# tbuckworth/train-procgen-pytorch

Hardware: AMD Instinct MI355X
Metric: env steps/sec (whole node), coinrun hard-500 IMPALA-CNN PPO (higher is better)
Workload: dtype bf16

## Files before the change

### scratch/kbench_cb.hip

```cpp
#include "conv_bf16.hip"
#include <cstdio>
#include <vector>
int main(int argc, char** argv) {
    const int n = argc > 1 ? atoi(argv[1]) : 8192, reps = 10;
    const size_t P = (size_t)n * 16 * 16 * 32, X = (size_t)n * 32 * 32 * 16;
    unsigned short *dp, *xi, *out, *bank; uint8_t* arg; float* slabs;
    hipMalloc(&dp, P * 2 + 4096); hipMalloc(&arg, P + 4096); hipMalloc(&xi, X * 2 + 4096); hipMalloc(&out, X * 2 + 4096);
    hipMalloc(&bank, 16 * 304 * 2 + 4096); hipMalloc(&slabs, (size_t)1024 * (4608 + 32) * 4);
    std::vector<unsigned short> h(X);
    for (size_t k = 0; k < X; ++k) h[k] = (unsigned short)((k * 2654435761u >> 16) & 0xBFFF);
    hipMemcpy(dp, h.data(), P * 2, hipMemcpyHostToDevice); hipMemcpy(xi, h.data(), X * 2, hipMemcpyHostToDevice);
    std::vector<uint8_t> ha(P);
    for (size_t k = 0; k < P; ++k) ha[k] = (uint8_t)((k * 40503u >> 7) % 9);
    hipMemcpy(arg, ha.data(), P, hipMemcpyHostToDevice);
    std::vector<unsigned short> hb(16 * 304, 0x3c00); hipMemcpy(bank, hb.data(), hb.size() * 2, hipMemcpyHostToDevice);
    hipStream_t st; hipStreamCreate(&st);
    hipEvent_t e0, e1; hipEventCreate(&e0); hipEventCreate(&e1);
    ConvArgs a{};
    a.in = dp; a.pool_arg = arg; a.out = out; a.n = n; a.bf16 = 1; a.wbank = bank; a.wg_in = xi; a.wg_partial = slabs;
    auto run = [&]() { launch_conv_dgrad_bf16(CS_16_32_32, a, st); };
    run(); hipStreamSynchronize(st);
#ifdef BF_TIMING
    unsigned long long zero[16] = {0}; hipMemcpyToSymbol(HIP_SYMBOL(g_bf_timing), zero, sizeof zero);
#endif
    hipEventRecord(e0, st);
    for (int r = 0; r < reps; ++r) run();
    hipEventRecord(e1, st); hipStreamSynchronize(st);
    float ms; hipEventElapsedTime(&ms, e0, e1);
    const int grid = conv_bwd_fused_grid(CS_16_32_32, n);
    printf("fused block2.conv backward n=%d grid=%d: %.1f us/launch  (%s)\n", n, grid, ms * 1000 / reps, hipGetErrorString(hipGetLastError()));
#ifdef BF_TIMING
    unsigned long long t[16]; hipMemcpyFromSymbol(t, HIP_SYMBOL(g_bf_timing), sizeof t);
    const char* nm[8] = {"top barrier (+ wait for loads)", "staging stores + barrier", "gather (+ next loads)", "barrier after gather", "wgrad MFMAs", "dgrad MFMAs", "tail: reduction + slab", "prologue"};
    for (int role = 0; role < 2; ++role)
        for (int k = 0; k < 8; ++k) printf("  wave %d %-32s %9.0f cycles/WG/launch (%.0f per item)\n", role * 4, nm[k], (double)t[role * 8 + k] / grid / reps, (double)t[role * 8 + k] / grid / reps / ((double)n * 4 / grid));
#endif
    return 0;
}
```

### train-procgen-pytorch_amd/csrc/conv_bf16.hip

```cpp
#include "common.h"
#include "device_util.h"
#include <mutex>
#include <type_traits>

static int c1_grid(int n);


template <int CH, int HO, int NPR>
struct PoolStage {
    static constexpr int NW = NPR * HO * (CH / 8), K = (NW + 255) / 256;
    static constexpr int PD_ELEMS = NPR * HO * CH;
    static constexpr size_t BYTES = (size_t)PD_ELEMS * 3;
    uint4 rd[K]; uint2 ra[K];
    __device__ __forceinline__ void load(const unsigned short* g_dp, const uint8_t* g_arg, long long img, int oyb) {
#pragma unroll
        for (int k = 0; k < K; ++k) {
            const int e = threadIdx.x + k * 256;
            rd[k] = (uint4){0u, 0u, 0u, 0u}; ra[k] = (uint2){0xffffffffu, 0xffffffffu};
            if (e < NW) {
                const int c8 = e % (CH / 8), ox = (e / (CH / 8)) % HO, oy = oyb + e / ((CH / 8) * HO);
                if (oy >= 0 && oy < HO) {
                    const long long o = ((img * HO + oy) * HO + ox) * CH + c8 * 8;
                    rd[k] = *(const uint4*)(g_dp + o); ra[k] = *(const uint2*)(g_arg + o);
                }
            }
        }
    }
    __device__ __forceinline__ void store(unsigned short* s_pd) const {
        uint8_t* s_pa = (uint8_t*)(s_pd + PD_ELEMS);
#pragma unroll
        for (int k = 0; k < K; ++k) {
            const int e = threadIdx.x + k * 256;
            if (e < NW) { *(uint4*)(s_pd + e * 8) = rd[k]; *(uint2*)(s_pa + e * 8) = ra[k]; }
        }
    }
    static __device__ __forceinline__ void gather(const unsigned short* s_pd, int a0, int y_lo, int y_hi, unsigned short* s_dst, int y_base,
                                                  int dst_pw, int xoff, int S) {
        for (int task = threadIdx.x; task < NTASK; task += 256) gather_task(s_pd, task, a0, y_lo, y_hi, s_dst, y_base, dst_pw, xoff, S);
    }
    static constexpr int NTASK = (NPR - 1) * HO * (CH / 4);
    static __device__ __forceinline__ void gather_task(const unsigned short* s_pd, int task, int a0, int y_lo, int y_hi, unsigned short* s_dst,
                                                       int y_base, int dst_pw, int xoff, int S) {
        const uint8_t* s_pa = (const uint8_t*)(s_pd + PD_ELEMS);
        constexpr int Q = CH / 4;
        {
            const int cq = task % Q, bx = (task / Q) % HO, bl = task / (Q * HO);
            float sm[4][4];
#pragma unroll
            for (int q = 0; q < 4; ++q)
#pragma unroll
                for (int c = 0; c < 4; ++c) sm[q][c] = 0.f;
#pragma unroll
            for (int wy = 0; wy < 2; ++wy)
#pragma unroll
                for (int wx = 0; wx < 2; ++wx) {
                    const int ox = bx + wx;
                    const int o = ((bl + wy) * HO + (ox < HO ? ox : HO - 1)) * CH + cq * 4;
                    const uint2 d = *(const uint2*)(s_pd + o);
                    unsigned ag = *(const unsigned*)(s_pa + o);
                    if (ox >= HO) ag = 0xffffffffu;
                    const float v[4] = {__uint_as_float(d.x << 16), __uint_as_float(d.x & 0xffff0000u), __uint_as_float(d.y << 16), __uint_as_float(d.y & 0xffff0000u)};
#pragma unroll
                    for (int dy = 0; dy < 2; ++dy)
#pragma unroll
                        for (int dx = 0; dx < 2; ++dx) {
                            const int ky = dy + 1 - 2 * wy, kx = dx + 1 - 2 * wx;
                            if (ky < 0 || kx < 0) continue;
                            const unsigned pos = (unsigned)(ky * 3 + kx);
#pragma unroll
                            for (int c = 0; c < 4; ++c)
                                sm[dy * 2 + dx][c] += (((ag >> (8 * c)) & 0xffu) == pos) ? v[c] : 0.f;
                        }
                }
#pragma unroll
            for (int dy = 0; dy < 2; ++dy) {
                const int y = 2 * (a0 + bl) + dy;
                if (y < y_lo || y >= y_hi) continue;
#pragma unroll
                for (int dx = 0; dx < 2; ++dx) {
                    const float* q = sm[dy * 2 + dx];
                    *(uint2*)(s_dst + ((y - y_base) * dst_pw + 2 * bx + dx + xoff) * S + cq * 4) =
                        (uint2){mi_pk_bf16(q[0], q[1]), mi_pk_bf16(q[2], q[3])};
                }
            }
        }
    }
    static constexpr int NTASK2 = (NPR - 1) * HO * (CH / 2);
    static __device__ __forceinline__ void gather_task2(const unsigned short* s_pd, int task, int a0, int y_lo, int y_hi, unsigned short* s_dst,
                                                        int y_base, int dst_pw, int xoff, int S) {
        const uint8_t* s_pa = (const uint8_t*)(s_pd + PD_ELEMS);
        constexpr int Q = CH / 2;
        const int cq = task % Q, bx = (task / Q) % HO, bl = task / (Q * HO);
        float sm[4][2];
#pragma unroll
        for (int q = 0; q < 4; ++q) { sm[q][0] = 0.f; sm[q][1] = 0.f; }
#pragma unroll
        for (int wy = 0; wy < 2; ++wy)
#pragma unroll
            for (int wx = 0; wx < 2; ++wx) {
                const int ox = bx + wx;
                const int o = ((bl + wy) * HO + (ox < HO ? ox : HO - 1)) * CH + cq * 2;
                const unsigned d = *(const unsigned*)(s_pd + o);
                unsigned ag = *(const unsigned short*)(s_pa + o);
                if (ox >= HO) ag = 0xffffu;
                const float v[2] = {__uint_as_float(d << 16), __uint_as_float(d & 0xffff0000u)};
#pragma unroll
                for (int dy = 0; dy < 2; ++dy)
#pragma unroll
                    for (int dx = 0; dx < 2; ++dx) {
                        const int ky = dy + 1 - 2 * wy, kx = dx + 1 - 2 * wx;
                        if (ky < 0 || kx < 0) continue;
                        const unsigned pos = (unsigned)(ky * 3 + kx);
#pragma unroll
                        for (int c = 0; c < 2; ++c)
                            sm[dy * 2 + dx][c] += (((ag >> (8 * c)) & 0xffu) == pos) ? v[c] : 0.f;
                    }
            }
#pragma unroll
        for (int dy = 0; dy < 2; ++dy) {
            const int y = 2 * (a0 + bl) + dy;
            if (y < y_lo || y >= y_hi) continue;
#pragma unroll
            for (int dx = 0; dx < 2; ++dx)
                *(unsigned*)(s_dst + ((y - y_base) * dst_pw + 2 * bx + dx + xoff) * S + cq * 2) = mi_pk_bf16(sm[dy * 2 + dx][0], sm[dy * 2 + dx][1]);
        }
    }
};

template <int CIN_, int COUT_, int HW_, int TH_, int TW_, int NIMG_, bool TRANSW_>
struct BfCfg {
    static constexpr int CIN = CIN_, COUT = COUT_, HW = HW_, TH = TH_, TW = TW_, NIMG = NIMG_;
    static constexpr bool TRANSW = TRANSW_;
    static constexpr int S = (CIN == 16) ? 16 : 48;
    static constexpr int PH = TH + 2, PW = TW + 2;
    static constexpr int NPIX = NIMG * PH * PW;
    static constexpr int IN_ELEMS = ((NPIX * S + 7) / 8) * 8;
    static constexpr int NK = (CIN == 32) ? 9 : 5;
    static constexpr int WS = NK * 32 + 16;
    static constexpr int W_ELEMS = COUT * WS;
    static constexpr int NMT = NIMG * TH * TW / 16, MT = NMT / 4, NB = COUT / 16;
    static constexpr int TPI_X = HW / TW, TPI = (HW / TH) * (HW / TW);
    static constexpr int C8 = CIN / 8;
    static constexpr int NLD = (NPIX * C8 + 255) / 256;
    static constexpr size_t LDS_BYTES = (size_t)(IN_ELEMS + W_ELEMS) * 2;
    static constexpr int WPE = 1;
    static_assert(NMT % 4 == 0, "M tiles must split over 4 waves");
};

template <class C>
__device__ __forceinline__ void bf_coords(int work, int& img0, int& ty0, int& tx0) {
    if (C::NIMG > 1) { img0 = work * C::NIMG; ty0 = 0; tx0 = 0; }
    else { img0 = work / C::TPI; const int t = work % C::TPI; ty0 = (t / C::TPI_X) * C::TH; tx0 = (t % C::TPI_X) * C::TW; }
}

template <class C>
__device__ __forceinline__ void bf_tile_load(uint4 (&r)[C::NLD], const unsigned short* in, int n_img, int img0, int ty0, int tx0) {
#pragma unroll
    for (int k = 0; k < C::NLD; ++k) {
        const int e = threadIdx.x + k * 256;
        uint4 v = {0u, 0u, 0u, 0u};
        if (e < C::NPIX * C::C8) {
            const int pix = e / C::C8, c8 = e % C::C8;
            const int img = pix / (C::PH * C::PW), q = pix % (C::PH * C::PW);
            const int gy = ty0 + q / C::PW - 1, gx = tx0 + q % C::PW - 1, n = img0 + img;
            if (n < n_img && gy >= 0 && gy < C::HW && gx >= 0 && gx < C::HW)
                v = *(const uint4*)(in + (((long long)n * C::HW + gy) * C::HW + gx) * C::CIN + c8 * 8);
        }
        r[k] = v;
    }
}
__device__ __forceinline__ unsigned relu_bf16x2(unsigned w) {
    const unsigned neg = (w >> 15) & 0x00010001u;
    return w & ~(neg * 0xFFFFu);
}
template <class C>
__device__ __forceinline__ void bf_tile_store(const uint4 (&r)[C::NLD], unsigned short* s_in, int relu_in) {
#pragma unroll
    for (int k = 0; k < C::NLD; ++k) {
        const int e = threadIdx.x + k * 256;
        if (e < C::NPIX * C::C8) {
            uint4 v = r[k];
            if (relu_in) { v.x = relu_bf16x2(v.x); v.y = relu_bf16x2(v.y); v.z = relu_bf16x2(v.z); v.w = relu_bf16x2(v.w); }
            *(uint4*)(s_in + (e / C::C8) * C::S + (e % C::C8) * 8) = v;
        }
    }
}

template <class C, bool POOLIN = false>
__global__ __launch_bounds__(256, C::WPE) void conv3x3_bf16_kernel(ConvArgs a) {
    extern __shared__ __attribute__((aligned(16))) unsigned short smem_h[];
    unsigned short* s_in = smem_h;
    unsigned short* s_w = smem_h + C::IN_ELEMS;
    using PS = PoolStage<C::CIN, C::HW / 2, C::TH / 2 + 3>;
    unsigned short* s_pd = s_w + C::W_ELEMS;
    static_assert(!POOLIN || (C::NIMG == 1 && C::TW == C::HW && C::TH % 2 == 0), "pooled input: full-width row tiles of one image");
    const int tid = threadIdx.x, lane = tid & 63, wave = tid >> 6;
    const int i = lane & 15, kq = lane >> 4;
    const unsigned short* g_in = (const unsigned short*)a.in;
    const unsigned short* g_mask = (const unsigned short*)a.mask;
    const unsigned short* g_res = (const unsigned short*)a.res;
    unsigned short* g_out = (unsigned short*)a.out;

    if (a.wbank) {
        for (int e = tid; e < C::COUT * C::WS / 8; e += 256) ((uint4*)s_w)[e] = ((const uint4*)a.wbank)[e];
    } else
    for (int e = tid; e < C::COUT * C::WS; e += 256) {
        const int j = e / C::WS, k = e % C::WS;
        float v = 0.f;
        const int tap = k / C::CIN, ci = k % C::CIN;
        if (k < C::NK * 32 && tap < 9) v = C::TRANSW ? a.w[(ci * 9 + (8 - tap)) * C::COUT + j] : a.w[(j * 9 + tap) * C::CIN + ci];
        s_w[e] = f2bf(v);
    }

    float bias_r[C::NB][4];
#pragma unroll
    for (int nb = 0; nb < C::NB; ++nb)
#pragma unroll
        for (int r = 0; r < 4; ++r) bias_r[nb][r] = a.bias ? a.bias[nb * 16 + kq * 4 + r] : 0.f;
    int koff[C::NK];
#pragma unroll
    for (int m = 0; m < C::NK; ++m) {
        int tap, chunk;
        if (C::CIN == 32) { tap = m; chunk = kq; } else { tap = 2 * m + (kq >> 1); chunk = kq & 1; if (tap > 8) tap = 8; }
        koff[m] = ((tap / 3) * C::PW + (tap % 3)) * C::S + chunk * 8;
    }

    const int nwork = (C::NIMG > 1) ? (a.n + C::NIMG - 1) / C::NIMG : a.n * C::TPI;
    uint4 regs[POOLIN ? 1 : C::NLD];
    PS ps;
    int img0, ty0, tx0;
    if (POOLIN) for (int e = tid; e < C::IN_ELEMS / 8; e += 256) ((uint4*)s_in)[e] = (uint4){0u, 0u, 0u, 0u};
    if ((int)blockIdx.x < nwork) {
        bf_coords<C>(blockIdx.x, img0, ty0, tx0);
        if constexpr (POOLIN) ps.load(g_in, a.pool_arg, img0, ty0 / 2 - 1); else bf_tile_load<C>(regs, g_in, a.n, img0, ty0, tx0);
    }
    for (int work = blockIdx.x; work < nwork; work += gridDim.x) {
        bf_coords<C>(work, img0, ty0, tx0);
        __syncthreads();
        if constexpr (POOLIN) {
            ps.store(s_pd);
            __syncthreads();
            PS::gather(s_pd, ty0 / 2 - 1, ty0 - 1, ty0 + C::TH + 1, s_in, ty0 - 1, C::PW, 1, C::S);
        } else bf_tile_store<C>(regs, s_in, a.relu_in);
        __syncthreads();
        if (work + (int)gridDim.x < nwork) {
            int i2, y2, x2;
            bf_coords<C>(work + gridDim.x, i2, y2, x2);
            if constexpr (POOLIN) ps.load(g_in, a.pool_arg, i2, y2 / 2 - 1); else bf_tile_load<C>(regs, g_in, a.n, i2, y2, x2);
        }
        uint2 e_mask[C::MT][C::NB], e_res[C::MT][C::NB];
        long long e_off[C::MT];
        bool e_on[C::MT];
#pragma unroll
        for (int mt = 0; mt < C::MT; ++mt) {
            const int pl = (wave * C::MT + mt) * 16 + i, y = pl / C::TW, x = pl % C::TW;
            int n = img0 + y / C::TH;
            e_on[mt] = n < a.n;
            n = n < a.n ? n : a.n - 1;
            e_off[mt] = (((long long)n * C::HW + ty0 + (y % C::TH)) * C::HW + tx0 + x) * C::COUT + kq * 4;
        }
        if (g_mask) {
#pragma unroll
            for (int mt = 0; mt < C::MT; ++mt)
#pragma unroll
                for (int nb = 0; nb < C::NB; ++nb) e_mask[mt][nb] = *(const uint2*)(g_mask + e_off[mt] + nb * 16);
        } else {
#pragma unroll
            for (int mt = 0; mt < C::MT; ++mt)
#pragma unroll
                for (int nb = 0; nb < C::NB; ++nb) e_mask[mt][nb] = (uint2){0x3f803f80u, 0x3f803f80u};
// ... 88 lines not shown
    const int i = lane & 15, kq = lane >> 4;
    const int pair = wave & 3, role = wave >> 2;
#ifdef BF_TIMING
    long long tacc_[8] = {0, 0, 0, 0, 0, 0, 0, 0}, tlast_ = clock64();
#endif
    const unsigned short* g_dp = (const unsigned short*)a.in;
    const unsigned short* g_xi = (const unsigned short*)a.wg_in;
    unsigned short* g_out = (unsigned short*)a.out;

    for (int e = tid; e < C::COUT * C::WS / 8; e += K::NT) ((uint4*)s_w)[e] = ((const uint4*)a.wbank)[e];
    for (int e = tid; e < K::IN_ELEMS / 8; e += K::NT) ((uint4*)s_in)[e] = (uint4){0u, 0u, 0u, 0u};
    for (int e = tid; e < K::XI_ELEMS / 8; e += K::NT) ((uint4*)s_xi)[e] = (uint4){0u, 0u, 0u, 0u};
    for (int e = tid; e < K::ONES_ELEMS / 2; e += K::NT) ((unsigned*)s_ones)[e] = 0x3f803f80u;

    uint4 rd, rxi[K::KXI]; uint2 ra;
    auto item_loads = [&](int work) {
        const int img = blockIdx.x + (work >> 2) * gridDim.x, k = work & 3, ty0 = k * 8;
        const int oy = 4 * k + tid / 64, oyc = oy < 16 ? oy : 15;
        const long long po = (((long long)img * 16 + oyc) * 16 * 4 + tid % 64) * 8;
        rd = *(const uint4*)(g_dp + po); ra = *(const uint2*)(a.pool_arg + po);
#pragma unroll
        for (int q = 0; q < K::KXI; ++q) {
            const int e = tid + q * K::NT, gy = ty0 - 1 + e / 64, gyc = gy < 0 ? 0 : (gy > 31 ? 31 : gy);
            rxi[q] = *(const uint4*)(g_xi + (((long long)img * 32 + gyc) * 64 + e % 64) * 8);
        }
    };
    f32x4 wacc[10];
#pragma unroll
    for (int k = 0; k < 10; ++k) wacc[k] = (f32x4){0.f, 0.f, 0.f, 0.f};
    const int cp = lane & 3;
    const int pl0 = 64 * pair + 16 * (kq >> 1) + 4 * (kq & 1) + ((lane & 15) >> 2);
    const int prow0 = (pl0 / 32) * C::PW + pl0 % 32;
    const unsigned short* dv_p = s_in + (prow0 + C::PW + 1) * C::S + 4 * cp;
    const unsigned short* xv_p = s_xi + prow0 * K::SX + 4 * cp;
    const unsigned short* av_p = s_in + (wave * C::PW + i) * C::S + kq * 8;
    const unsigned short* bv_p = s_w + i * C::WS + kq * 8;
    const int ooff = (wave * 32 + i) * 16 + kq * 4;
    const unsigned short* xvp[5];
#pragma unroll
    for (int sl = 0; sl < 5; ++sl) {
        const int tap = role ? 5 + sl : sl;
        xvp[sl] = (role && sl == 4) ? s_ones : xv_p + ((tap / 3) * C::PW + tap % 3) * K::SX;
    }
    auto wg_steps = [&]() {
#pragma unroll
        for (int st = 0; st < 2; ++st) {
            bf16x8 dv[2];
#pragma unroll
            for (int cb = 0; cb < 2; ++cb) {
                const s16x4 lo = __builtin_amdgcn_ds_read_tr16_b64_v4i16((lds_s16x4_ptr)(dv_p + st * C::PW * C::S + cb * 16));
                const s16x4 hi = __builtin_amdgcn_ds_read_tr16_b64_v4i16((lds_s16x4_ptr)(dv_p + (st * C::PW + 8) * C::S + cb * 16));
                dv[cb] = __builtin_shufflevector(lo, hi, 0, 1, 2, 3, 4, 5, 6, 7);
            }
#pragma unroll
            for (int sl = 0; sl < 5; ++sl) {
                const s16x4 lo = __builtin_amdgcn_ds_read_tr16_b64_v4i16((lds_s16x4_ptr)(xvp[sl] + st * C::PW * K::SX));
                const s16x4 hi = __builtin_amdgcn_ds_read_tr16_b64_v4i16((lds_s16x4_ptr)(xvp[sl] + (st * C::PW + 8) * K::SX));
                const bf16x8 xv = __builtin_shufflevector(lo, hi, 0, 1, 2, 3, 4, 5, 6, 7);
#pragma unroll
                for (int cb = 0; cb < 2; ++cb) wacc[sl * 2 + cb] = MFMA_BF16(dv[cb], xv, wacc[sl * 2 + cb]);
            }
        }
    };

    const int nwork = 4 * ((a.n - (int)blockIdx.x + (int)gridDim.x - 1) / (int)gridDim.x);
    item_loads(0);
    B2CK(7);
    uint2 ost[2] = {(uint2){0u, 0u}, (uint2){0u, 0u}}; unsigned short* ob = g_out;
    for (int work = 0; work < nwork; ++work) {
        const int img = blockIdx.x + (work >> 2) * gridDim.x, k = work & 3, ty0 = k * 8;
        __syncthreads();
        __builtin_amdgcn_s_waitcnt(0x0F70);
        B2CK(0);
        if (k) { for (int e = tid; e < 3 * K::ROW_WORDS; e += K::NT) ((uint4*)s_in)[e] = ((const uint4*)s_in)[8 * K::ROW_WORDS + e]; }
        else if (tid < K::ROW_WORDS) ((uint4*)s_in)[tid] = (uint4){0u, 0u, 0u, 0u};
        if (tid < PS::NW) {
            const bool in = 4 * k + tid / 64 < 16;
            *(uint4*)(s_pd + tid * 8) = in ? rd : (uint4){0u, 0u, 0u, 0u};
            *(uint2*)((uint8_t*)(s_pd + PS::PD_ELEMS) + tid * 8) = in ? ra : (uint2){0xffffffffu, 0xffffffffu};
        }
#pragma unroll
        for (int q = 0; q < K::KXI; ++q) {
            const int e = tid + q * K::NT, gy = ty0 - 1 + e / 64;
            if (e < K::NXI) *(uint4*)(s_xi + ((e / 64) * C::PW + (e / 2) % 32 + 1) * K::SX + (e % 2) * 8) = (gy >= 0 && gy < 32) ? rxi[q] : (uint4){0u, 0u, 0u, 0u};
        }
        if (work) { *(uint2*)(ob + ooff) = ost[0]; *(uint2*)(ob + ooff + 256) = ost[1]; }
        __syncthreads();
        B2CK(1);
#pragma unroll 1
        for (int task = tid + (k ? 256 : 0); task < PS::NTASK2; task += K::NT) PS::gather_task2(s_pd, task, 4 * k, -1000, 1000, s_in, ty0 - 1, C::PW, 1, C::S);
        item_loads(work + 1 < nwork ? work + 1 : work);
        B2CK(2);
        __syncthreads();
        B2CK(3);
        wg_steps();
        B2CK(4);
        f32x4 acc[2] = {(f32x4){0.f, 0.f, 0.f, 0.f}, (f32x4){0.f, 0.f, 0.f, 0.f}};
#pragma unroll
        for (int m = 0; m < 9; ++m) {
            const bf16x8 bv = *(const bf16x8*)(bv_p + m * 32);
#pragma unroll
            for (int mt = 0; mt < 2; ++mt) acc[mt] = MFMA_BF16(bv, *(const bf16x8*)(av_p + ((m / 3) * C::PW + (m % 3) + 16 * mt) * C::S), acc[mt]);
        }
        B2CK(5);
        ob = g_out + ((long long)img * 32 + ty0) * 32 * 16;
#pragma unroll
        for (int mt = 0; mt < 2; ++mt) ost[mt] = (uint2){mi_pk_bf16(acc[mt][0], acc[mt][1]), mi_pk_bf16(acc[mt][2], acc[mt][3])};
    }
    if (nwork > 0) { *(uint2*)(ob + ooff) = ost[0]; *(uint2*)(ob + ooff + 256) = ost[1]; }
    __syncthreads();
    float* red = (float*)smem_h;
    float* redb = red + K::WLEN;
    for (int w = 0; w < 4; ++w) {
        if (pair == w) {
#pragma unroll
            for (int sl = 0; sl < 5; ++sl)
#pragma unroll
                for (int cb = 0; cb < 2; ++cb)
#pragma unroll
                    for (int r = 0; r < 4; ++r) {
                        const float v = wacc[sl * 2 + cb][r];
                        if (role && sl == 4) { if (i == 0) { const int o = cb * 16 + kq * 4 + r; redb[o] = (w == 0) ? v : redb[o] + v; } }
                        else {
                            const int tap = role ? 5 + sl : sl;
                            const int o = ((cb * 16 + kq * 4 + r) * 9 + tap) * 16 + i;
                            red[o] = (w == 0) ? v : red[o] + v;
                        }
                    }
        }
        __syncthreads();
    }
    float* slab = a.wg_partial + (long long)blockIdx.x * K::SLAB;
    for (int e = tid; e < K::SLAB; e += K::NT) slab[e] = red[e];
#ifdef BF_TIMING
    B2CK(6);
    if ((threadIdx.x & 255) == 0) for (int q = 0; q < 8; ++q) atomicAdd(&g_bf_timing[(threadIdx.x >> 8) * 8 + q], (unsigned long long)tacc_[q]);
#endif
}
static int b2bwd_grid(int n) { return n > 512 ? 512 : n; }
static void launch_block2_conv_bwd(const ConvArgs& a, hipStream_t st) {
    static std::once_flag attr;
    std::call_once(attr, [] { hipFuncSetAttribute((const void*)block2_conv_bwd_bf16_kernel, hipFuncAttributeMaxDynamicSharedMemorySize, (int)B2Bwd::LDS); });
    const int grid = b2bwd_grid(a.n);
    if (grid < 1) return;
    hipLaunchKernelGGL(block2_conv_bwd_bf16_kernel, dim3(grid), dim3(B2Bwd::NT), B2Bwd::LDS, st, a);
}

struct B3Bwd {
    using PS = PoolStage<32, 8, 9>;
    static constexpr int NT = 512, NIMG = 2, HW = 16, P = HW + 2, S = 48;
    static constexpr int T_ELEMS = P * P * S;
    static constexpr int PD_ALL = PS::PD_ELEMS + (PS::PD_ELEMS + 1) / 2;
    static constexpr int WS = 9 * 32 + 16, WLEN = 32 * 9 * 32, SLAB = WLEN + 32;
    static constexpr int NMT = NIMG * HW * HW / 16, NSTEP = NIMG * HW * HW / 32;
    static constexpr size_t LDS = (size_t)NIMG * (2 * T_ELEMS + PD_ALL) * 2;
    static_assert(LDS <= 160 * 1024 && PD_ALL % 8 == 0, "one workgroup per CU; 16-byte aligned stages");
    static_assert(PS::NTASK2 == 1024, "two gather tasks per thread and image");
};
__global__ __launch_bounds__(512, 2) void block3_conv_bwd_bf16_kernel(ConvArgs a) {
    using K = B3Bwd; using PS = K::PS;
    extern __shared__ __attribute__((aligned(16))) unsigned short smem_h[];
    unsigned short* s_dc = smem_h;
    unsigned short* s_xi = s_dc + K::NIMG * K::T_ELEMS;
    unsigned short* s_pd = s_xi + K::NIMG * K::T_ELEMS;
    const int tid = threadIdx.x, lane = tid & 63, i = lane & 15, kq = lane >> 4, rq = (lane & 15) >> 2, cp = lane & 3;
    const int wv = __builtin_amdgcn_readfirstlane(tid >> 6);
    const bool conv_role = wv < 4;
    const int rw = wv & 3;
    const unsigned short* g_dp = (const unsigned short*)a.in;
    const unsigned short* g_xi = (const unsigned short*)a.wg_in;
    unsigned short* g_out = (unsigned short*)a.out;
    for (int e = tid; e < (int)(K::LDS / 16); e += K::NT) ((uint4*)smem_h)[e] = (uint4){0u, 0u, 0u, 0u};
    __syncthreads();
    for (int e = tid; e < K::NIMG * 8 * 32; e += K::NT)
        ((uint8_t*)(s_pd + (e >> 8) * K::PD_ALL + PS::PD_ELEMS))[8 * 8 * 32 + (e & 255)] = 0xff;
    constexpr int NST = 22, QM = 5;
    f32x4 st[NST];
    const int qcnt = (18 - rw + 3) / 4;
    if (conv_role) {
#pragma unroll
        for (int m = 0; m < 9; ++m)
#pragma unroll
            for (int nb = 0; nb < 2; ++nb) st[2 * m + nb] = __builtin_bit_cast(f32x4, *(const uint4*)(a.wbank + (nb * 16 + i) * K::WS + m * 32 + kq * 8));
#pragma unroll
        for (int q = 18; q < NST; ++q) st[q] = (f32x4){0.f, 0.f, 0.f, 0.f};
    } else {
#pragma unroll
        for (int q = 0; q < NST; ++q) st[q] = (f32x4){0.f, 0.f, 0.f, 0.f};
    }
    __builtin_amdgcn_s_waitcnt(0x0F70);
    const bf16x8 ones = __builtin_bit_cast(bf16x8, (uint4){0x3f803f80u, 0x3f803f80u, 0x3f803f80u, 0x3f803f80u});
    auto koffc = [](int m) { return ((m / 3) * K::P + (m % 3)) * K::S; };
    auto porg = [](int pl) { return (pl >> 8) * K::T_ELEMS + (((pl >> 4) & 15) * K::P + (pl & 15)) * K::S; };
    constexpr int CENTER = (K::P + 1) * K::S;

    const int nwork = (a.n + K::NIMG - 1) / K::NIMG;
    typedef unsigned b3_u32x4 __attribute__((ext_vector_type(4)));
    typedef unsigned b3_u32x2 __attribute__((ext_vector_type(2)));
    b3_u32x4 rx[4], rg; b3_u32x2 ra;
    auto load = [&](int work) {
        const int img0 = work * K::NIMG;
#pragma unroll
        for (int k = 0; k < 4; ++k) {
            const int e = tid + k * K::NT, pl = e >> 2;
            const int n = img0 + (pl >> 8) < a.n ? img0 + (pl >> 8) : a.n - 1;
            rx[k] = *(const b3_u32x4*)(g_xi + ((long long)n * 256 + (pl & 255)) * 32 + (e & 3) * 8);
        }
        const int n = img0 + (tid >> 8) < a.n ? img0 + (tid >> 8) : a.n - 1;
        const long long o = (long long)n * 2048 + (tid & 255) * 8;
        rg = *(const b3_u32x4*)(g_dp + o); ra = *(const b3_u32x2*)(a.pool_arg + o);
    };
    auto wg_step = [&](int t) {
        int orow[2];
#pragma unroll
        for (int h = 0; h < 2; ++h) orow[h] = porg(32 * t + 16 * (kq >> 1) + 8 * h + 4 * (kq & 1) + rq) + 4 * cp;
        auto tr = [&](const unsigned short* base, int off) {
            const s16x4 lo = __builtin_amdgcn_ds_read_tr16_b64_v4i16((lds_s16x4_ptr)(base + orow[0] + off));
            const s16x4 hi = __builtin_amdgcn_ds_read_tr16_b64_v4i16((lds_s16x4_ptr)(base + orow[1] + off));
            return (bf16x8)__builtin_shufflevector(lo, hi, 0, 1, 2, 3, 4, 5, 6, 7);
        };
        bf16x8 d[2], b[QM];
#pragma unroll
        for (int cb = 0; cb < 2; ++cb) d[cb] = tr(s_dc, CENTER + cb * 16);
#pragma unroll
        for (int qq = 0; qq < QM; ++qq) {
            const int q = rw + 4 * (qq < 4 ? qq : (qcnt > 4 ? 4 : 0)), tap = q >> 1, ib = q & 1;
            b[qq] = tr(s_xi, koffc(tap) + ib * 16);
        }
        asm volatile("" ::: "memory");
        if (rw == 2) { st[20] = MFMA_BF16(d[0], ones, st[20]); st[21] = MFMA_BF16(d[1], ones, st[21]); }
#pragma unroll
        for (int qq = 0; qq < QM; ++qq)
            if (qq < qcnt) {
#pragma unroll
                for (int cb = 0; cb < 2; ++cb) st[2 * qq + cb] = MFMA_BF16(d[cb], b[qq], st[2 * qq + cb]);
            }
    };

    if ((int)blockIdx.x < nwork) load(blockIdx.x);
    for (int work = blockIdx.x; work < nwork; work += gridDim.x) {
        const int img0 = work * K::NIMG, left = a.n - img0;
        __syncthreads();
        {
            const b3_u32x4 z = {0u, 0u, 0u, 0u};
#pragma unroll
            for (int k = 0; k < 4; ++k) {
                const int e = tid + k * K::NT, pl = e >> 2;
                *(b3_u32x4*)(s_xi + porg(pl) + CENTER + (e & 3) * 8) = (pl >> 8) < left ? rx[k] : z;
            }
            unsigned short* pd = s_pd + (tid >> 8) * K::PD_ALL;
            *(b3_u32x4*)(pd + (tid & 255) * 8) = (tid >> 8) < left ? rg : z;
            *(b3_u32x2*)((uint8_t*)(pd + PS::PD_ELEMS) + (tid & 255) * 8) = ra;
        }
        __syncthreads();
#pragma unroll
        for (int im = 0; im < K::NIMG; ++im)
#pragma unroll
            for (int j = 0; j < 2; ++j)
                PS::gather_task2(s_pd + im * K::PD_ALL, tid + j * K::NT, 0, -1000, 1000, s_dc + im * K::T_ELEMS, -1, K::P, 1, K::S);
        if (work + (int)gridDim.x < nwork) load(work + gridDim.x);
        __syncthreads();
        if (conv_role) {
            for (int t = rw; t < K::NMT; t += 4) {
                const int pl = t * 16 + i;
                const unsigned short* src = s_dc + porg(pl) + kq * 8;
                bf16x8 av[5];
#pragma unroll
                for (int m = 0; m < 5; ++m) av[m] = *(const bf16x8*)(src + koffc(m));
                asm volatile("" ::: "memory");
                f32x4 acc[2] = {{0.f, 0.f, 0.f, 0.f}, {0.f, 0.f, 0.f, 0.f}};
#pragma unroll
                for (int m = 0; m < 9; ++m) {
                    const bf16x8 cur = av[m % 5];
                    acc[0] = MFMA_BF16(__builtin_bit_cast(bf16x8, st[2 * m]), cur, acc[0]);
                    acc[1] = MFMA_BF16(__builtin_bit_cast(bf16x8, st[2 * m + 1]), cur, acc[1]);
                    if (m < 4) av[m] = *(const bf16x8*)(src + koffc(m + 5));
                }
                if ((pl >> 8) < left) {
#pragma unroll
                    for (int nb = 0; nb < 2; ++nb)
                        *(uint2*)(g_out + ((long long)img0 * 256 + pl) * 32 + nb * 16 + kq * 4) =
                            (uint2){mi_pk_bf16(acc[nb][0], acc[nb][1]), mi_pk_bf16(acc[nb][2], acc[nb][3])};
                }
            }
        } else {
#pragma unroll 4
            for (int t = 0; t < K::NSTEP; ++t) wg_step(t);
        }
    }
    if (!conv_role) {
        float* sl = a.wg_partial + (long long)blockIdx.x * K::SLAB;
#pragma unroll
        for (int qq = 0; qq < QM; ++qq)
            if (qq < qcnt) {
                const int q = rw + 4 * qq, tap = q >> 1, ib = q & 1;
#pragma unroll
                for (int cb = 0; cb < 2; ++cb)
#pragma unroll
                    for (int r = 0; r < 4; ++r) sl[((cb * 16 + kq * 4 + r) * 9 + tap) * 32 + ib * 16 + i] = st[2 * qq + cb][r];
            }
        if (i == 0 && rw == 2) {
#pragma unroll
            for (int cb = 0; cb < 2; ++cb)
#pragma unroll
                for (int r = 0; r < 4; ++r) sl[K::WLEN + cb * 16 + kq * 4 + r] = st[20 + cb][r];
        }
    }
}
static int b3bwd_grid(int n) { const int w = (n + B3Bwd::NIMG - 1) / B3Bwd::NIMG; return w > 256 ? 256 : w; }
static void launch_block3_conv_bwd(const ConvArgs& a, hipStream_t st) {
    static std::once_flag attr;
    std::call_once(attr, [] { hipFuncSetAttribute((const void*)block3_conv_bwd_bf16_kernel, hipFuncAttributeMaxDynamicSharedMemorySize, (int)B3Bwd::LDS); });
    const int grid = b3bwd_grid(a.n);
    if (grid < 1) return;
    hipLaunchKernelGGL(block3_conv_bwd_bf16_kernel, dim3(grid), dim3(B3Bwd::NT), B3Bwd::LDS, st, a);
}

int bank_ws(int cin_pass) { return (cin_pass == 32 ? 9 : 5) * 32 + 16; }
__global__ void pack_banks_kernel(const float* __restrict__ params, unsigned short* __restrict__ banks, const BankDesc* __restrict__ desc) {
    const BankDesc d = desc[blockIdx.y];
    const float* w = params + d.w_off;
    unsigned short* out = banks + d.out_off;
    for (int e = blockIdx.x * blockDim.x + threadIdx.x; e < d.rows * d.ws; e += gridDim.x * blockDim.x) {
        const int j = e / d.ws, k = e % d.ws, tap = k / d.cin_pass, ci = k % d.cin_pass;
        float v = 0.f;
        if (k < d.nk * 32 && tap < 9) v = d.transw ? w[(ci * 9 + (8 - tap)) * d.ci_f + j] : w[(j * 9 + tap) * d.ci_f + ci];
        out[e] = f2bf(v);
    }
}
void launch_pack_banks(const float* params, unsigned short* banks, const BankDesc* d_desc, int n_desc, hipStream_t st) {
    if (n_desc <= 0) return;
    hipLaunchKernelGGL(pack_banks_kernel, dim3(8, n_desc), dim3(256), 0, st, params, banks, d_desc);
}

#ifndef WG_WPE
#define WG_WPE 2
#endif
#ifndef WG16_TH
#define WG16_TH 16
#endif
#ifndef WG8_NIMG
#define WG8_NIMG 4
#endif

template <int CIN_, int COUT_, int HW_, int TH_, int TW_, int NIMG_>
struct WbCfg {
    static constexpr int CIN = CIN_, COUT = COUT_, HW = HW_, TH = TH_, TW = TW_, NIMG = NIMG_;
    static constexpr int S = (CIN == 16) ? 16 : 48, SO = (COUT == 16) ? 16 : 48;
    static constexpr int PH = TH + 2, PW = TW + 2, NPIX = NIMG * PH * PW, NT = NIMG * TH * TW;
    static constexpr int IN_ELEMS = ((NPIX * S + 7) / 8) * 8, DO_ELEMS = ((NT * SO + 7) / 8) * 8;
    static constexpr int NCB = COUT / 16, NIB = CIN / 16, NSTEP = NT / 32;
    static constexpr int WLEN = COUT * 9 * CIN, SLAB = WLEN + COUT;
    static constexpr int C8 = CIN / 8, OC8 = COUT / 8;
    static constexpr int NLD = (NPIX * C8 + 255) / 256, NDO = (NT * OC8 + 255) / 256;
    static constexpr int TPI_X = HW / TW, TPI = (HW / TH) * (HW / TW);
    static constexpr bool SPLIT = (CIN == 32 && COUT == 32);
    static constexpr int NQ = 9 * NIB, QMAX = (NQ + 3) / 4;
    static constexpr size_t TILE_BYTES = (size_t)(IN_ELEMS + DO_ELEMS) * 2, RED_BYTES = (size_t)((SPLIT ? 0 : WLEN) + 256) * 4;
    static constexpr size_t LDS_BYTES = TILE_BYTES > RED_BYTES ? TILE_BYTES : RED_BYTES;
    static_assert(NT % 32 == 0, "pixel steps of 32");
};

#ifdef WG_TIMING
__device__ unsigned long long g_wg_timing[8];
#define TCK(k) do { if (tid == 0) { const long long now_ = clock64(); tacc_[k] += now_ - tlast_; tlast_ = now_; } } while (0)
#else
#define TCK(k) do { } while (0)
#endif

template <class C, bool POOLED = false>
__global__ __launch_bounds__(256, C::SPLIT ? WG_WPE : 1) void conv3x3_wgrad_bf16_kernel(WgradArgs a) {
    extern __shared__ __attribute__((aligned(16))) unsigned short smem_h[];
    using PS = PoolStage<C::COUT, C::HW / 2, C::TH / 2 + 1>;
    static_assert(!POOLED || (C::NIMG == 1 && C::TW == C::HW && C::TH % 2 == 0), "pooled dOut: full-width row tiles of one image");
    PS ps;
#ifdef WG_TIMING
    long long tacc_[8] = {0, 0, 0, 0, 0, 0, 0, 0}, tlast_ = clock64();
#endif
    unsigned short* s_in = smem_h;
    unsigned short* s_do = smem_h + C::IN_ELEMS;
    const int tid = threadIdx.x, lane = tid & 63, wave = tid >> 6;
    const int i = lane & 15, kq = lane >> 4, rq = (lane & 15) >> 2, cp = lane & 3;
    const unsigned short* g_in = (const unsigned short*)a.in;
    const unsigned short* g_do = (const unsigned short*)a.dout;
    constexpr int NACC = C::SPLIT ? C::QMAX * C::NCB : 9 * C::NCB * C::NIB;
    f32x4 acc[NACC];
#pragma unroll
    for (int k = 0; k < NACC; ++k) acc[k] = (f32x4){0.f, 0.f, 0.f, 0.f};
    const int wv = __builtin_amdgcn_readfirstlane(wave);
    const int qcnt = (C::NQ - wv + 3) / 4;
    f32x4 accb[C::NCB];
#pragma unroll
    for (int cb = 0; cb < C::NCB; ++cb) accb[cb] = (f32x4){0.f, 0.f, 0.f, 0.f};
    const bf16x8 ones = __builtin_bit_cast(bf16x8, (uint4){0x3f803f80u, 0x3f803f80u, 0x3f803f80u, 0x3f803f80u});

    const int nwork = (C::NIMG > 1) ? (a.n + C::NIMG - 1) / C::NIMG : a.n * C::TPI;
    uint4 rin[C::NLD], rdo[C::NDO];
    int ioff[C::TPI == 1 ? C::NLD : 1], doff[C::TPI == 1 ? C::NDO : 1];
    if constexpr (C::TPI == 1) {
#pragma unroll
        for (int k = 0; k < C::NLD; ++k) {
            const int e = tid + k * 256;
            ioff[k] = -1;
            if (e < C::NPIX * C::C8) {
                const int pix = e / C::C8, c8 = e % C::C8, img = pix / (C::PH * C::PW), q = pix % (C::PH * C::PW);
                const int gy = q / C::PW - 1, gx = q % C::PW - 1;
                if (gy >= 0 && gy < C::HW && gx >= 0 && gx < C::HW) ioff[k] = ((img * C::HW + gy) * C::HW + gx) * C::CIN + c8 * 8;
            }
        }
#pragma unroll
        for (int k = 0; k < C::NDO; ++k) {
            const int e = tid + k * 256;
            doff[k] = -1;
            if (e < C::NT * C::OC8) {
                const int pl = e / C::OC8, c8 = e % C::OC8, y = pl / C::TW, x = pl % C::TW;
                doff[k] = (((y / C::TH) * C::HW + (y % C::TH)) * C::HW + x) * C::COUT + c8 * 8;
            }
        }
    }
    auto coords = [&](int work, int& img0, int& ty0, int& tx0) {
        if (C::NIMG > 1) { img0 = work * C::NIMG; ty0 = 0; tx0 = 0; }
        else { img0 = work / C::TPI; const int t = work % C::TPI; ty0 = (t / C::TPI_X) * C::TH; tx0 = (t % C::TPI_X) * C::TW; }
    };
    auto load = [&](int img0, int ty0, int tx0) {
        if constexpr (C::TPI == 1) {
            const int left = a.n - img0;
            const unsigned short* bi = g_in + (long long)img0 * (C::HW * C::HW * C::CIN);
            const unsigned short* bd = g_do + (long long)img0 * (C::HW * C::HW * C::COUT);
#pragma unroll
            for (int k = 0; k < C::NLD; ++k) {
                uint4 v = {0u, 0u, 0u, 0u};
                if (ioff[k] >= 0 && (C::NIMG == 1 || ioff[k] / (C::HW * C::HW * C::CIN) < left)) v = *(const uint4*)(bi + ioff[k]);
                rin[k] = v;
            }
            if constexpr (POOLED) ps.load(g_do, a.pool_arg, img0, ty0 / 2);
            else {
#pragma unroll
                for (int k = 0; k < C::NDO; ++k) {
                    uint4 v = {0u, 0u, 0u, 0u};
                    if (doff[k] >= 0 && (C::NIMG == 1 || doff[k] / (C::HW * C::HW * C::COUT) < left)) v = *(const uint4*)(bd + doff[k]);
                    rdo[k] = v;
                }
// ... 837 lines not shown
```

Baseline: 722,300.

## Software-pipeline block3 conv backward per image with role-specialized load/gather stages

Result: no change. 724,400 (median of 3 runs) (+0.3%).

```diff
diff --git a/scratch/kbench_cb.hip b/scratch/kbench_cb.hip
--- a/scratch/kbench_cb.hip
+++ b/scratch/kbench_cb.hip
@@ -1,6 +1,7 @@
 #include "conv_bf16.hip"
 #include <cstdio>
 #include <vector>
+void mi_launch_fail(const char* msg) { fprintf(stderr, "%s\n", msg); }
 int main(int argc, char** argv) {
     const int n = argc > 1 ? atoi(argv[1]) : 8192, reps = 10;
     const size_t P = (size_t)n * 16 * 16 * 32, X = (size_t)n * 32 * 32 * 16;
diff --git a/scratch/kbench_cb3.hip b/scratch/kbench_cb3.hip
--- /dev/null
+++ b/scratch/kbench_cb3.hip
@@ -0,0 +1,42 @@
+#include "conv_bf16.hip"
+#include <cstdio>
+#include <vector>
+void mi_launch_fail(const char* msg) { fprintf(stderr, "%s\n", msg); }
+int main(int argc, char** argv) {
+    const int n = argc > 1 ? atoi(argv[1]) : 8192, reps = 10;
+    const size_t P = (size_t)n * 8 * 8 * 32, X = (size_t)n * 16 * 16 * 32;
+    unsigned short *dp, *xi, *out, *bank; uint8_t* arg; float* slabs;
+    hipMalloc(&dp, P * 2 + 4096); hipMalloc(&arg, P + 4096); hipMalloc(&xi, X * 2 + 4096); hipMalloc(&out, X * 2 + 4096);
+    hipMalloc(&bank, 32 * 304 * 2 + 4096); hipMalloc(&slabs, (size_t)1024 * (9216 + 32) * 4);
+    std::vector<unsigned short> h(X);
+    for (size_t k = 0; k < X; ++k) h[k] = (unsigned short)((k * 2654435761u >> 16) & 0xBFFF);
+    hipMemcpy(dp, h.data(), P * 2, hipMemcpyHostToDevice); hipMemcpy(xi, h.data(), X * 2, hipMemcpyHostToDevice);
+    std::vector<uint8_t> ha(P);
+    for (size_t k = 0; k < P; ++k) ha[k] = (uint8_t)((k * 40503u >> 7) % 9);
+    hipMemcpy(arg, ha.data(), P, hipMemcpyHostToDevice);
+    std::vector<unsigned short> hb(32 * 304, 0x3c00); hipMemcpy(bank, hb.data(), hb.size() * 2, hipMemcpyHostToDevice);
+    hipStream_t st; hipStreamCreate(&st);
+    hipEvent_t e0, e1; hipEventCreate(&e0); hipEventCreate(&e1);
+    ConvArgs a{};
+    a.in = dp; a.pool_arg = arg; a.out = out; a.n = n; a.bf16 = 1; a.wbank = bank; a.wg_in = xi; a.wg_partial = slabs;
+    auto run = [&]() { launch_conv_dgrad_bf16(CS_32_32_16, a, st); };
+    run(); hipStreamSynchronize(st);
+#ifdef BF_TIMING
+    unsigned long long zero[16] = {0}; hipMemcpyToSymbol(HIP_SYMBOL(g_bf_timing), zero, sizeof zero);
+#endif
+    hipEventRecord(e0, st);
+    for (int r = 0; r < reps; ++r) run();
+    hipEventRecord(e1, st); hipStreamSynchronize(st);
+    float ms; hipEventElapsedTime(&ms, e0, e1);
+    const int grid = conv_bwd_fused_grid(CS_32_32_16, n);
+    printf("fused block3.conv backward n=%d grid=%d: %.1f us/launch  (%s)\n", n, grid, ms * 1000 / reps, hipGetErrorString(hipGetLastError()));
+#ifdef BF_TIMING
+    unsigned long long t[16]; hipMemcpyFromSymbol(t, HIP_SYMBOL(g_bf_timing), sizeof t);
+    const char* nm[8] = {"staging stores (+ wait for loads)", "gather of the next image", "MFMAs of this image", "barrier", "-", "-", "tail: slab", "prologue"};
+    const char* role[2] = {"conv role (wave 0)", "wgrad role (wave 4)"};
+    for (int r = 0; r < 2; ++r)
+        for (int k = 0; k < 8; ++k)
+            if (nm[k][0] != '-') printf("  %-20s %-34s %9.0f cycles/WG/launch (%.0f per image)\n", role[r], nm[k], (double)t[r * 8 + k] / grid / reps, (double)t[r * 8 + k] / reps / n);
+#endif
+    return 0;
+}
diff --git a/train-procgen-pytorch_amd/csrc/conv_bf16.hip b/train-procgen-pytorch_amd/csrc/conv_bf16.hip
--- a/train-procgen-pytorch_amd/csrc/conv_bf16.hip
+++ b/train-procgen-pytorch_amd/csrc/conv_bf16.hip
@@ -88,10 +88,14 @@
     static constexpr int NTASK2 = (NPR - 1) * HO * (CH / 2);
     static __device__ __forceinline__ void gather_task2(const unsigned short* s_pd, int task, int a0, int y_lo, int y_hi, unsigned short* s_dst,
                                                         int y_base, int dst_pw, int xoff, int S) {
+        float sm[4][2];
+        gather_sum2(s_pd, task, sm);
+        gather_put2(sm, task, a0, y_lo, y_hi, s_dst, y_base, dst_pw, xoff, S);
+    }
+    static __device__ __forceinline__ void gather_sum2(const unsigned short* s_pd, int task, float (&sm)[4][2]) {
         const uint8_t* s_pa = (const uint8_t*)(s_pd + PD_ELEMS);
         constexpr int Q = CH / 2;
         const int cq = task % Q, bx = (task / Q) % HO, bl = task / (Q * HO);
-        float sm[4][2];
 #pragma unroll
         for (int q = 0; q < 4; ++q) { sm[q][0] = 0.f; sm[q][1] = 0.f; }
 #pragma unroll
@@ -116,6 +120,11 @@
                             sm[dy * 2 + dx][c] += (((ag >> (8 * c)) & 0xffu) == pos) ? v[c] : 0.f;
                     }
             }
+    }
+    static __device__ __forceinline__ void gather_put2(const float (&sm)[4][2], int task, int a0, int y_lo, int y_hi, unsigned short* s_dst,
+                                                       int y_base, int dst_pw, int xoff, int S) {
+        constexpr int Q = CH / 2;
+        const int cq = task % Q, bx = (task / Q) % HO, bl = task / (Q * HO);
 #pragma unroll
         for (int dy = 0; dy < 2; ++dy) {
             const int y = 2 * (a0 + bl) + dy;
@@ -510,10 +519,10 @@
     static constexpr int T_ELEMS = P * P * S;
     static constexpr int PD_ALL = PS::PD_ELEMS + (PS::PD_ELEMS + 1) / 2;
     static constexpr int WS = 9 * 32 + 16, WLEN = 32 * 9 * 32, SLAB = WLEN + 32;
-    static constexpr int NMT = NIMG * HW * HW / 16, NSTEP = NIMG * HW * HW / 32;
+    static constexpr int NMT = HW * HW / 16, NSTEP = HW * HW / 32;
     static constexpr size_t LDS = (size_t)NIMG * (2 * T_ELEMS + PD_ALL) * 2;
     static_assert(LDS <= 160 * 1024 && PD_ALL % 8 == 0, "one workgroup per CU; 16-byte aligned stages");
-    static_assert(PS::NTASK2 == 1024, "two gather tasks per thread and image");
+    static_assert(NIMG == 2 && PS::NTASK2 == 4 * (NT / 2) && 8 * 8 * 32 / 8 == NT / 2, "four gather tasks per conv-role thread and image; one pooled-stage word per weight-gradient thread");
 };
 __global__ __launch_bounds__(512, 2) void block3_conv_bwd_bf16_kernel(ConvArgs a) {
     using K = B3Bwd; using PS = K::PS;
@@ -525,6 +534,9 @@
     const int wv = __builtin_amdgcn_readfirstlane(tid >> 6);
     const bool conv_role = wv < 4;
     const int rw = wv & 3;
+#ifdef BF_TIMING
+    long long tacc_[8] = {0, 0, 0, 0, 0, 0, 0, 0}, tlast_ = clock64();
+#endif
     const unsigned short* g_dp = (const unsigned short*)a.in;
     const unsigned short* g_xi = (const unsigned short*)a.wg_in;
     unsigned short* g_out = (unsigned short*)a.out;
@@ -549,26 +561,49 @@
     __builtin_amdgcn_s_waitcnt(0x0F70);
     const bf16x8 ones = __builtin_bit_cast(bf16x8, (uint4){0x3f803f80u, 0x3f803f80u, 0x3f803f80u, 0x3f803f80u});
     auto koffc = [](int m) { return ((m / 3) * K::P + (m % 3)) * K::S; };
-    auto porg = [](int pl) { return (pl >> 8) * K::T_ELEMS + (((pl >> 4) & 15) * K::P + (pl & 15)) * K::S; };
+    auto porg = [](int pl) { return (((pl >> 4) & 15) * K::P + (pl & 15)) * K::S; };
     constexpr int CENTER = (K::P + 1) * K::S;
 
     const int nwork = (a.n + K::NIMG - 1) / K::NIMG;
+    int nseq = 0;
+    if ((int)blockIdx.x < nwork) {
+        const int rounds = (nwork - (int)blockIdx.x + (int)gridDim.x - 1) / (int)gridDim.x, last = blockIdx.x + (rounds - 1) * gridDim.x;
+        nseq = 2 * rounds - (2 * last + 1 < a.n ? 0 : 1);
+    }
+    auto img_of = [&](int s) { const int im = 2 * ((int)blockIdx.x + (s >> 1) * (int)gridDim.x) + (s & 1); return im < a.n ? im : a.n - 1; };
     typedef unsigned b3_u32x4 __attribute__((ext_vector_type(4)));
     typedef unsigned b3_u32x2 __attribute__((ext_vector_type(2)));
+    const int ts = tid - 256;
     b3_u32x4 rx[4], rg; b3_u32x2 ra;
-    auto load = [&](int work) {
-        const int img0 = work * K::NIMG;
+    auto load_x = [&](int s) {
+        const unsigned short* src = g_xi + (long long)img_of(s) * (256 * 32);
+#pragma unroll
+        for (int k = 0; k < 4; ++k) rx[k] = *(const b3_u32x4*)(src + (ts + k * 256) * 8);
+    };
+    auto store_x = [&](int slot) {
 #pragma unroll
         for (int k = 0; k < 4; ++k) {
-            const int e = tid + k * K::NT, pl = e >> 2;
-            const int n = img0 + (pl >> 8) < a.n ? img0 + (pl >> 8) : a.n - 1;
-            rx[k] = *(const b3_u32x4*)(g_xi + ((long long)n * 256 + (pl & 255)) * 32 + (e & 3) * 8);
-        }
-        const int n = img0 + (tid >> 8) < a.n ? img0 + (tid >> 8) : a.n - 1;
-        const long long o = (long long)n * 2048 + (tid & 255) * 8;
+            const int e = ts + k * 256;
+            *(b3_u32x4*)(s_xi + slot * K::T_ELEMS + porg(e >> 2) + CENTER + (e & 3) * 8) = rx[k];
+        }
+    };
+    auto load_p = [&](int s) {
+        const long long o = (long long)img_of(s) * 2048 + ts * 8;
         rg = *(const b3_u32x4*)(g_dp + o); ra = *(const b3_u32x2*)(a.pool_arg + o);
     };
-    auto wg_step = [&](int t) {
+    auto store_p = [&](int slot) {
+        unsigned short* pd = s_pd + slot * K::PD_ALL;
+        *(b3_u32x4*)(pd + ts * 8) = rg;
+        *(b3_u32x2*)((uint8_t*)(pd + PS::PD_ELEMS) + ts * 8) = ra;
+    };
+    auto gather = [&](int slot) {
+        float sm[4][4][2];
+#pragma unroll
+        for (int j = 0; j < 4; ++j) PS::gather_sum2(s_pd + slot * K::PD_ALL, tid + j * 256, sm[j]);
+#pragma unroll
+        for (int j = 0; j < 4; ++j) PS::gather_put2(sm[j], tid + j * 256, 0, -1000, 1000, s_dc + slot * K::T_ELEMS, -1, K::P, 1, K::S);
+    };
+    auto wg_step = [&](const unsigned short* s_dc, const unsigned short* s_xi, int t) {
         int orow[2];
 #pragma unroll
         for (int h = 0; h < 2; ++h) orow[h] = porg(32 * t + 16 * (kq >> 1) + 8 * h + 4 * (kq & 1) + rq) + 4 * cp;
@@ -595,33 +630,29 @@
             }
     };
 
-    if ((int)blockIdx.x < nwork) load(blockIdx.x);
-    for (int work = blockIdx.x; work < nwork; work += gridDim.x) {
-        const int img0 = work * K::NIMG, left = a.n - img0;
-        __syncthreads();
-        {
-            const b3_u32x4 z = {0u, 0u, 0u, 0u};
-#pragma unroll
-            for (int k = 0; k < 4; ++k) {
-                const int e = tid + k * K::NT, pl = e >> 2;
-                *(b3_u32x4*)(s_xi + porg(pl) + CENTER + (e & 3) * 8) = (pl >> 8) < left ? rx[k] : z;
-            }
-            unsigned short* pd = s_pd + (tid >> 8) * K::PD_ALL;
-            *(b3_u32x4*)(pd + (tid & 255) * 8) = (tid >> 8) < left ? rg : z;
-            *(b3_u32x2*)((uint8_t*)(pd + PS::PD_ELEMS) + (tid & 255) * 8) = ra;
-        }
-        __syncthreads();
-#pragma unroll
-        for (int im = 0; im < K::NIMG; ++im)
-#pragma unroll
-            for (int j = 0; j < 2; ++j)
-                PS::gather_task2(s_pd + im * K::PD_ALL, tid + j * K::NT, 0, -1000, 1000, s_dc + im * K::T_ELEMS, -1, K::P, 1, K::S);
-        if (work + (int)gridDim.x < nwork) load(work + gridDim.x);
-        __syncthreads();
-        if (conv_role) {
-            for (int t = rw; t < K::NMT; t += 4) {
+    if (nseq > 0) {
+        if (!conv_role) {
+            load_x(0); load_p(0);
+            store_x(0); store_p(0);
+            load_x(1); load_p(1);
+        }
+        __syncthreads();
+        if (conv_role) gather(0);
+        else { store_p(1); load_p(2); }
+        __syncthreads();
+    }
+    B2CK(7);
+    if (conv_role) {
+        for (int s = 0; s < nseq; ++s) {
+            const int slot = s & 1;
+            if (s + 1 < nseq) gather(slot ^ 1);
+            B2CK(1);
+            const long long img = 2 * ((long long)blockIdx.x + (s >> 1) * (long long)gridDim.x) + slot;
+#pragma unroll
+            for (int tt = 0; tt < 4; ++tt) {
+                const int t = rw + 4 * tt;
                 const int pl = t * 16 + i;
-                const unsigned short* src = s_dc + porg(pl) + kq * 8;
+                const unsigned short* src = s_dc + slot * K::T_ELEMS + porg(pl) + kq * 8;
                 bf16x8 av[5];
 #pragma unroll
                 for (int m = 0; m < 5; ++m) av[m] = *(const bf16x8*)(src + koffc(m));
@@ -634,18 +665,31 @@
                     acc[1] = MFMA_BF16(__builtin_bit_cast(bf16x8, st[2 * m + 1]), cur, acc[1]);
                     if (m < 4) av[m] = *(const bf16x8*)(src + koffc(m + 5));
                 }
-                if ((pl >> 8) < left) {
-#pragma unroll
-                    for (int nb = 0; nb < 2; ++nb)
-                        *(uint2*)(g_out + ((long long)img0 * 256 + pl) * 32 + nb * 16 + kq * 4) =
-                            (uint2){mi_pk_bf16(acc[nb][0], acc[nb][1]), mi_pk_bf16(acc[nb][2], acc[nb][3])};
-                }
-            }
-        } else {
+#pragma unroll
+                for (int nb = 0; nb < 2; ++nb)
+                    *(uint2*)(g_out + (img * 256 + pl) * 32 + nb * 16 + kq * 4) =
+                        (uint2){mi_pk_bf16(acc[nb][0], acc[nb][1]), mi_pk_bf16(acc[nb][2], acc[nb][3])};
+            }
+            B2CK(2);
+            __syncthreads();
+            B2CK(3);
+        }
+    } else {
+        for (int s = 0; s < nseq; ++s) {
+            const int slot = s & 1;
+            store_x(slot ^ 1); store_p(slot);
+            load_x(s + 2); load_p(s + 3);
+            B2CK(0);
 #pragma unroll 4
-            for (int t = 0; t < K::NSTEP; ++t) wg_step(t);
-        }
-    }
+            for (int t = 0; t < K::NSTEP; ++t) wg_step(s_dc + slot * K::T_ELEMS, s_xi + slot * K::T_ELEMS, t);
+            B2CK(2);
+            __syncthreads();
+            B2CK(3);
+        }
+    }
+#ifdef BF_TIMING
+    if ((threadIdx.x & 255) == 0) for (int q = 0; q < 8; ++q) atomicAdd(&g_bf_timing[(threadIdx.x >> 8) * 8 + q], (unsigned long long)tacc_[q]);
+#endif
     if (!conv_role) {
         float* sl = a.wg_partial + (long long)blockIdx.x * K::SLAB;
 #pragma unroll
```
